# JasperSnoek/spearmint

Hardware: NVIDIA H100
Metric: EI candidates/sec (higher is better)
Workload: dtype f32

## Files before the change

### spearmint_b200/csrc/predict_tc.cu

```cuda
#include <cuda_fp16.h>
#include <cuda.h>

#include <algorithm>
#include <vector>
#include <cstdlib>
#include <cstring>

#include "common.cuh"
#include "tc_common.cuh"

namespace smk {

__global__ void __launch_bounds__(256, 2) trtri_finalize_kernel(int Npad, int ldx, int K, const float* __restrict__ winv,
                                                                 float* X) {
  using C = Cfg<float>;
  constexpr int NB = C::NB, TM = C::TM, TN = C::TN;
  extern __shared__ __align__(16) unsigned char smem_raw[];
  TileSmem<float>& sm = *reinterpret_cast<TileSmem<float>*>(smem_raw);
  float (*Ts)[NB + kPad] = reinterpret_cast<float (*)[NB + kPad]>(smem_raw + sizeof(TileSmem<float>));
  const int nblk = Npad / NB, J = blockIdx.x, s = blockIdx.y;
  const int tid = threadIdx.x, ty = tid >> 4, tx = tid & 15;
  const float* W = winv + ((long)s * nblk + K) * NB * NB;
  float* Xt = X + (long)s * ldx * ldx + (long)K * NB * ldx + (long)J * NB;
  float acc[TM][TN];
  if (J == K) {
#pragma unroll
    for (int r = 0; r < TM; ++r)
#pragma unroll
      for (int g = 0; g < TN / 4; ++g) {
        V4<float> v = ld4(W + (long)tile_row(ty, r) * NB + g * 64 + tx * 4);
#pragma unroll
        for (int e = 0; e < 4; ++e) acc[r][g * 4 + e] = v.v[e];
      }
  } else {
#pragma unroll
    for (int r = 0; r < TM; ++r)
#pragma unroll
      for (int g = 0; g < TN / 4; ++g) {
        V4<float> v = ld4(Xt + (long)tile_row(ty, r) * ldx + g * 64 + tx * 4);
        st4(&Ts[tile_row(ty, r)][g * 64 + tx * 4], v);
      }
#pragma unroll
    for (int r = 0; r < TM; ++r)
#pragma unroll
      for (int c = 0; c < TN; ++c) acc[r][c] = 0.f;
    TileGemm<float, Lay::KContig, Lay::MContig, false>::run_bsmem(acc, W, NB, &Ts[0][0], NB + kPad, NB, sm);
  }
#pragma unroll
  for (int r = 0; r < TM; ++r)
#pragma unroll
    for (int g = 0; g < TN / 4; ++g) {
      V4<float> v;
#pragma unroll
      for (int e = 0; e < 4; ++e) v.v[e] = acc[r][g * 4 + e];
      st4(Xt + (long)tile_row(ty, r) * ldx + g * 64 + tx * 4, v);
    }
}

__global__ void __launch_bounds__(256, 2) trtri_update_kernel(int Npad, int ldx, int K, const float* __restrict__ L,
                                                               float* X) {
  using C = Cfg<float>;
  constexpr int NB = C::NB, TM = C::TM, TN = C::TN;
  __shared__ TileSmem<float> sm;
  const int I = K + 1 + blockIdx.x, J = blockIdx.y, s = blockIdx.z;
  const int tid = threadIdx.x, ty = tid >> 4, tx = tid & 15;
  const float* Lik = L + (long)s * Npad * Npad + (long)I * NB * Npad + (long)K * NB;
  float* Xs = X + (long)s * ldx * ldx;
  float* Xij = Xs + (long)I * NB * ldx + (long)J * NB;
  const float* Xkj = Xs + (long)K * NB * ldx + (long)J * NB;
  float acc[TM][TN];
  if (K == J) {
#pragma unroll
    for (int r = 0; r < TM; ++r)
#pragma unroll
      for (int c = 0; c < TN; ++c) acc[r][c] = 0.f;
  } else {
#pragma unroll
    for (int r = 0; r < TM; ++r)
#pragma unroll
      for (int g = 0; g < TN / 4; ++g) {
        V4<float> v = ld4(Xij + (long)tile_row(ty, r) * ldx + g * 64 + tx * 4);
#pragma unroll
        for (int e = 0; e < 4; ++e) acc[r][g * 4 + e] = v.v[e];
      }
  }
  TileGemm<float, Lay::KContig, Lay::MContig, true>::run(acc, Lik, Npad, Xkj, ldx, NB, sm);
#pragma unroll
  for (int r = 0; r < TM; ++r)
#pragma unroll
    for (int g = 0; g < TN / 4; ++g) {
      V4<float> v;
#pragma unroll
      for (int e = 0; e < 4; ++e) v.v[e] = acc[r][g * 4 + e];
      st4(Xij + (long)tile_row(ty, r) * ldx + g * 64 + tx * 4, v);
    }
}

__device__ __forceinline__ float tf32_hi(float x) { return tf32_rn(x); }

__global__ void split_lower_kernel(int Npad, int ld, long total, const float* __restrict__ X, float* __restrict__ hi,
                                   float* __restrict__ lo) {
  long e = (long)blockIdx.x * blockDim.x + threadIdx.x;
  if (e >= total) return;
  long per = (long)ld * ld;
  int r = (int)((e % per) / ld), c = (int)(e % ld);
  float x = (c <= r && r < Npad) ? X[e] : 0.f;
  float h = tf32_hi(x);
  hi[e] = h;
  lo[e] = x - h;
}

__global__ void __launch_bounds__(256) linv_mv_kernel(int N, int Np, const float* __restrict__ hi,
                                                      const float* __restrict__ lo, const float* __restrict__ y,
                                                      const float* __restrict__ mean, float* __restrict__ t) {
  const int s = blockIdx.y, warp = threadIdx.x >> 5, lane = threadIdx.x & 31;
  const int row = blockIdx.x * 8 + warp;
  if (row >= Np) return;
  const long base = ((long)s * Np + row) * Np;
  const float mu = mean[s];
  float acc = 0.f;
  for (int k = lane; k <= row && k < N; k += 32) acc = fmaf(hi[base + k] + lo[base + k], y[k] - mu, acc);
#pragma unroll
  for (int o = 16; o > 0; o >>= 1) acc += __shfl_xor_sync(0xffffffffu, acc, o);
  if (lane == 0) t[(long)s * Np + row] = (row < N) ? acc : 0.f;
}
__global__ void __launch_bounds__(256) linv_mtv_kernel(int N, int Np, int ld_alpha, const float* __restrict__ hi,
                                                       const float* __restrict__ lo, const float* __restrict__ t,
                                                       float* __restrict__ alpha) {
  __shared__ float red[4][64];
  const int s = blockIdx.y, cl = threadIdx.x & 63, ph = threadIdx.x >> 6;
  const int c = blockIdx.x * 64 + cl;
  const float* th = t + (long)s * Np;
  const long base = (long)s * Np * Np + c;
  float acc = 0.f;
  if (c < N)
    for (int r = (c & ~3) + ph; r < N; r += 4)
      if (r >= c) acc = fmaf(hi[base + (long)r * Np] + lo[base + (long)r * Np], th[r], acc);
  red[ph][cl] = acc;
  __syncthreads();
  if (ph == 0 && c < ld_alpha) alpha[(long)s * ld_alpha + c] = (c < N) ? red[0][cl] + red[1][cl] + red[2][cl] + red[3][cl] : 0.f;
}

__global__ void __launch_bounds__(256) linv_absmax_kernel(long per4, const float4* __restrict__ hi,
                                                          const float4* __restrict__ lo, unsigned* __restrict__ maxbits) {
  const int s = blockIdx.y;
  const float4* h = hi + (long)s * per4;
  const float4* l = lo + (long)s * per4;
  float m = 0.f;
  for (long e = (long)blockIdx.x * blockDim.x + threadIdx.x; e < per4; e += (long)gridDim.x * blockDim.x) {
    float4 a = h[e], b = l[e];
    m = fmaxf(m, fmaxf(fmaxf(fabsf(a.x + b.x), fabsf(a.y + b.y)), fmaxf(fabsf(a.z + b.z), fabsf(a.w + b.w))));
  }
#pragma unroll
  for (int o = 16; o > 0; o >>= 1) m = fmaxf(m, __shfl_xor_sync(0xffffffffu, m, o));
  if ((threadIdx.x & 31) == 0) atomicMax(&maxbits[s], __float_as_uint(m));
}

__global__ void __launch_bounds__(256) linv_pack_f16_kernel(long per4, const float4* __restrict__ hi,
                                                            const float4* __restrict__ lo,
                                                            const unsigned* __restrict__ maxbits, uint2* __restrict__ oh,
                                                            uint2* __restrict__ ol, int* __restrict__ exps) {
  const int s = blockIdx.y;
  const int eb = scale_exp(__uint_as_float(maxbits[s]));
  const float sc = ldexpf(1.f, eb);
  if (blockIdx.x == 0 && threadIdx.x == 0) exps[s] = eb;
  const long base = (long)s * per4;
  for (long e = (long)blockIdx.x * blockDim.x + threadIdx.x; e < per4; e += (long)gridDim.x * blockDim.x) {
    float4 a = hi[base + e], b = lo[base + e];
    __half hh[4], ll[4];
    split16((a.x + b.x) * sc, hh[0], ll[0]);
    split16((a.y + b.y) * sc, hh[1], ll[1]);
    split16((a.z + b.z) * sc, hh[2], ll[2]);
    split16((a.w + b.w) * sc, hh[3], ll[3]);
    oh[base + e] = pack4(hh);
    ol[base + e] = pack4(ll);
  }
}

__global__ void __launch_bounds__(256) alpha_absmax_kernel(int N, int F, int Npad_alpha, const float* __restrict__ alpha,
                                                           int* __restrict__ fexp) {
  __shared__ float red[8];
  const int s = blockIdx.x;
  float m = 0.f;
  for (long e = threadIdx.x; e < (long)F * N; e += blockDim.x) {
    int f = (int)(e / N), n = (int)(e % N);
    m = fmaxf(m, fabsf(alpha[((long)s * F + f) * Npad_alpha + n]));
  }
#pragma unroll
  for (int o = 16; o > 0; o >>= 1) m = fmaxf(m, __shfl_xor_sync(0xffffffffu, m, o));
  if ((threadIdx.x & 31) == 0) red[threadIdx.x >> 5] = m;
  __syncthreads();
  if (threadIdx.x == 0) {
    for (int w = 1; w < 8; ++w) m = fmaxf(m, red[w]);
    fexp[s] = scale_exp(m);
  }
}
__global__ void alpha_pack_f16_kernel(int N, int Np, int F, int Fp, int Npad_alpha, long total,
                                      const float* __restrict__ alpha, const int* __restrict__ fexp,
                                      __half* __restrict__ hi, __half* __restrict__ lo) {
  long e = (long)blockIdx.x * blockDim.x + threadIdx.x;
  if (e >= total) return;
  int n = (int)(e % Np);
  long sf = e / Np;
  int f = (int)(sf % Fp), s = (int)(sf / Fp);
  float x = (f < F && n < N) ? alpha[((long)s * F + f) * Npad_alpha + n] * ldexpf(1.f, fexp[s]) : 0.f;
  split16(x, hi[e], lo[e]);
}

constexpr int kKD = 16;

__global__ void __launch_bounds__(256, 2) kxt_kernel(int kind, int N, int Np, int M, int c_begin, int Mc, int D,
                                                     const float* __restrict__ X, const float* __restrict__ Cc,
                                                     const float* __restrict__ inv_ls, const float* __restrict__ amp2,
                                                     const float* __restrict__ mean, const float* __restrict__ alpha,
                                                     int Npad_alpha, __half* __restrict__ khi,
                                                     __half* __restrict__ klo, float* __restrict__ mu, int ldm) {
  constexpr int T = 128, LDC = T + kPad, LDX = T + kPad;
  __shared__ __align__(16) float cs[kKD][LDC];
  __shared__ __align__(16) float xs[kKD][LDX];
  __shared__ __align__(16) float red[16][T];
  static_assert((LDC * sizeof(float)) % 16 == 0 && (LDX * sizeof(float)) % 16 == 0, "128-bit shared loads");
  const int s = blockIdx.y, c0 = blockIdx.x * T;
  const int tid = threadIdx.x, ty = tid >> 4, tx = tid & 15;
  const float* ils = inv_ls + (long)s * D;
  const float a2 = amp2[s];
  const float2 a2s = dup2(a2 * ldexpf(1.f, kx_exp(a2)));
  const float* al = alpha ? alpha + (long)s * Npad_alpha : nullptr;
  float2 mdot[8];
#pragma unroll
  for (int r = 0; r < 8; ++r) mdot[r] = make_float2(0.f, 0.f);

  for (int n0 = 0; n0 < Np; n0 += T) {
    float2 acc[8][4];
#pragma unroll
    for (int r = 0; r < 8; ++r)
#pragma unroll
      for (int c = 0; c < 4; ++c) acc[r][c] = make_float2(0.f, 0.f);
    for (int d0 = 0; d0 < D; d0 += kKD) {
      __syncthreads();
      for (int e = tid; e < T * kKD; e += 256) {
        int row = e / kKD, dd = e % kKD, d = d0 + dd;
        int gc = min(c_begin + c0 + row, M - 1), n = n0 + row;
        float sc = (d < D) ? ils[d] : 0.f;
        cs[dd][row] = (d < D) ? Cc[(long)gc * D + d] * sc : 0.f;
        xs[dd][row] = (d < D && n < N) ? -X[(long)n * D + d] * sc : 0.f;
      }
      __syncthreads();
      const int dmax = min(kKD, D - d0);
      for (int dd = 0; dd < dmax; ++dd) {
        float2 b[4];
#pragma unroll
        for (int g = 0; g < 2; ++g) {
          const V4<float> u = ld4(&xs[dd][g * 64 + tx * 4]);
          b[2 * g] = make_float2(u.v[0], u.v[1]);
          b[2 * g + 1] = make_float2(u.v[2], u.v[3]);
        }
#pragma unroll
        for (int g = 0; g < 2; ++g) {
          const float4 p0 = *reinterpret_cast<const float4*>(&cs[dd][g * 64 + ty * 4]);
          const float2 a[4] = {dup2(p0.x), dup2(p0.y), dup2(p0.z), dup2(p0.w)};
#pragma unroll
          for (int rr = 0; rr < 4; ++rr)
#pragma unroll
            for (int c = 0; c < 4; ++c) {
              const float2 df = fadd2(a[rr], b[c]);
              acc[g * 4 + rr][c] = ffma2(df, df, acc[g * 4 + rr][c]);
            }
        }
      }
    }
    const bool edge = (n0 + T > N);
    float2 av[4];
#pragma unroll
    for (int c = 0; c < 4; ++c) {
      const int n = n0 + (c >> 1) * 64 + tx * 4 + (c & 1) * 2;
      av[c] = al ? make_float2((n < N) ? al[n] : 0.f, (n + 1 < N) ? al[n + 1] : 0.f) : make_float2(0.f, 0.f);
    }
#pragma unroll
    for (int r = 0; r < 8; ++r) {
      const long ok = ((long)s * Mc + c0 + tile_row(ty, r)) * Np + n0;
#pragma unroll
      for (int g = 0; g < 2; ++g) {
        __half2 hh[2], ll[2];
#pragma unroll
        for (int q = 0; q < 2; ++q) {
          const int c = 2 * g + q;
          float2 kk = kernel_pair_fast(kind, acc[r][c]);
          if (edge) {
            const int n = n0 + g * 64 + tx * 4 + q * 2;
            if (n >= N) kk.x = 0.f;
            if (n + 1 >= N) kk.y = 0.f;
          }
          mdot[r] = ffma2(av[c], kk, mdot[r]);
          const float2 v = fmul2(kk, a2s);
          hh[q] = __floats2half2_rn(v.x, v.y);
          const float2 hf = __half22float2(hh[q]);
          ll[q] = __floats2half2_rn(v.x - hf.x, v.y - hf.y);
        }
        uint2 ph, pl;
        ph.x = *reinterpret_cast<unsigned*>(&hh[0]); ph.y = *reinterpret_cast<unsigned*>(&hh[1]);
        pl.x = *reinterpret_cast<unsigned*>(&ll[0]); pl.y = *reinterpret_cast<unsigned*>(&ll[1]);
        *reinterpret_cast<uint2*>(khi + ok + g * 64 + tx * 4) = ph;
        *reinterpret_cast<uint2*>(klo + ok + g * 64 + tx * 4) = pl;
      }
    }
  }
  if (!al) return;
  __syncthreads();
#pragma unroll
  for (int r = 0; r < 8; ++r) red[tx][tile_row(ty, r)] = mdot[r].x + mdot[r].y;
  __syncthreads();
  if (tid < T) {
    float v = 0.f;
    for (int q = 0; q < 16; ++q) v += red[q][tid];
    int gc = c_begin + c0 + tid;
    if (gc < M) mu[(long)s * ldm + gc] = fmaf(a2, v, mean[s]);
  }
}

namespace tc {
constexpr int BM = 128;
constexpr int BN = 256;
constexpr int BK = 16;
constexpr int BK16 = 32;
constexpr int STAGES = 4;
constexpr int ROW_BYTES = BK * 4;
static_assert(ROW_BYTES == 64 && BK16 * 2 == ROW_BYTES, "operand rows must be one 64B swizzle span in both element types");
constexpr int UK_BYTES = 32;
constexpr int A_BYTES = BM * ROW_BYTES;
constexpr int B_BYTES = BN * ROW_BYTES;
constexpr int STAGE_BYTES = 2 * A_BYTES + 2 * B_BYTES;
constexpr int CONSUMERS = 2;
constexpr int THREADS = (CONSUMERS + 1) * 128;
constexpr int PRODUCER_REGS = 40, CONSUMER_REGS = 232;
static_assert(128 * PRODUCER_REGS + CONSUMERS * 128 * CONSUMER_REGS <= 65536, "register file");
constexpr int SMEM_BYTES = STAGES * STAGE_BYTES + 1024  + 256 ;

struct Args {
  int S, Np, Mc, ntiles, npairs, ngroups, ldp;
  float* partial;
  const float* z;
  float* mpartial;
  float* dbg;
  int F, M, c_begin, ldm;
  const float* mean;
  float* mu_f;
  int f16;
  int a_evict_first;
  const float* amp2;
  const int* bexp;
  int mode;
  int Npad, jb, ncols;
  float* Cmat;
  int K;
  float *xhi, *xlo, *xthi, *xtlo;
};

struct Item { int valid, own, rowA, rowB, k0, nk, s, tile, g, pr; };

template <int CLUSTER>
__device__ __forceinline__ long num_items(const Args& p) {
  return p.mode <= 1 ? (long)p.S * ((p.ntiles + CLUSTER - 1) / CLUSTER) * p.npairs : (long)p.S * p.ntiles;
}
template <int CLUSTER>
__device__ __forceinline__ Item get_item(const Args& p, long w, int h, int rank) {
  Item it;
  it.valid = 0; it.own = 1; it.rowA = it.rowB = it.k0 = it.nk = it.s = it.tile = it.g = it.pr = 0;
  const int bk = p.f16 ? BK16 : BK;
  if (p.mode <= 1) {
    const int ntg = (p.ntiles + CLUSTER - 1) / CLUSTER;
    it.pr = (int)(w % p.npairs);
    const long st = w / p.npairs;
    it.tile = (int)(st % ntg) * CLUSTER + rank;
    it.s = (int)(st / ntg);
    if (it.tile >= p.ntiles) { it.tile = p.ntiles - 1; it.own = 0; }
    it.g = (h == 0) ? it.pr : p.ngroups - 1 - it.pr;
    if (h == 1 && (p.mode == 1 || it.g == it.pr)) return it;
    it.nk = (p.mode == 1) ? p.Np / bk : (it.g + 1) * (BN / bk);
    it.rowA = it.s * p.Mc + it.tile * BM;
    it.rowB = (it.s * p.ngroups + it.g) * BN;
    it.valid = 1;
  } else if (p.mode == 2) {
    if (h == 1) return it;
    it.tile = (int)(w % p.ntiles);
    it.s = (int)(w / p.ntiles);
    it.rowA = it.s * p.Npad + (p.jb + it.tile) * BM;
    it.rowB = it.s * p.Npad + p.jb * BM;
    it.nk = p.jb * BM / bk;
    it.valid = 1;
  } else {
    if (h == 1) return it;
    it.tile = (int)(w % p.ntiles);
    it.s = (int)(w / p.ntiles);
    it.rowA = it.s * BM;
    it.rowB = it.s * p.Np + it.tile * BN;
    it.k0 = it.tile * BN;
    it.nk = (p.K * BM - it.tile * BN) / bk;
    it.valid = 1;
  }
  return it;
}

template <int CLUSTER>
__global__ void __launch_bounds__(THREADS, 1)
predict_tc_kernel(const __grid_constant__ CUtensorMap mAhi, const __grid_constant__ CUtensorMap mAlo,
                  const __grid_constant__ CUtensorMap mBhi, const __grid_constant__ CUtensorMap mBlo, Args p) {
  static_assert(CLUSTER == 1 || CLUSTER == 2, "one CTA, or a pair sharing the B operand");
  extern __shared__ unsigned char smem_raw[];
  unsigned char* base = smem_raw + ((1024u - (smem_u32(smem_raw) & 1023u)) & 1023u);
  uint64_t* bars = reinterpret_cast<uint64_t*>(base + STAGES * STAGE_BYTES);
  uint64_t* full = bars;
  uint64_t* empty = bars + STAGES;

  const int warp = threadIdx.x >> 5, lane = threadIdx.x & 31;
  const int rank = CLUSTER > 1 ? (int)cluster_ctarank() : 0;
  if (threadIdx.x == 0) {
    for (int i = 0; i < STAGES; ++i) { mbar_init(&full[i], 1); mbar_init(&empty[i], CLUSTER * CONSUMERS * 4); }
    asm volatile("fence.mbarrier_init.release.cluster;" ::: "memory");
  }
  if (CLUSTER > 1) cluster_sync();
  else __syncthreads();

  const long nitems = num_items<CLUSTER>(p);
  const long w0 = blockIdx.x / CLUSTER, dw = gridDim.x / CLUSTER;
  const int bk = p.f16 ? BK16 : BK;
  if (warp < 4) {
    asm volatile("setmaxnreg.dec.sync.aligned.u32 %0;" ::"n"(PRODUCER_REGS));
    if (warp == 0 && lane == 0) {
      const uint64_t hintA = (p.mode == 0 && !p.a_evict_first) ? 0x1000000000000000ull : 0x12F0000000000000ull;
      const uint64_t hintB = 0x14F0000000000000ull;
      int stage = 0;
      uint32_t phase = 0;
      for (long w = w0; w < nitems; w += dw) {
        for (int h = 0; h < 2; ++h) {
          const Item it = get_item<CLUSTER>(p, w, h, rank);
          if (!it.valid) break;
          for (int kc = 0; kc < it.nk; ++kc) {
            mbar_wait_relaxed(&empty[stage], phase ^ 1, 64);
            unsigned char* sb = base + stage * STAGE_BYTES;
            const int kk = it.k0 + kc * bk;
            mbar_expect_tx(&full[stage], STAGE_BYTES);
            tma_load_2d(&mAhi, &full[stage], sb, kk, it.rowA, hintA);
            tma_load_2d(&mAlo, &full[stage], sb + A_BYTES, kk, it.rowA, hintA);
            if (CLUSTER == 1) {
              tma_load_2d(&mBhi, &full[stage], sb + 2 * A_BYTES, kk, it.rowB, hintB);
              tma_load_2d(&mBlo, &full[stage], sb + 2 * A_BYTES + B_BYTES, kk, it.rowB, hintB);
            } else {
              const int hb = rank * (BN / CLUSTER);
              const uint16_t all = (1u << CLUSTER) - 1;
              tma_load_2d_multicast(&mBhi, &full[stage], sb + 2 * A_BYTES + hb * ROW_BYTES, kk, it.rowB + hb, all, hintB);
              tma_load_2d_multicast(&mBlo, &full[stage], sb + 2 * A_BYTES + B_BYTES + hb * ROW_BYTES, kk, it.rowB + hb,
                                    all, hintB);
            }
            if (++stage == STAGES) { stage = 0; phase ^= 1; }
          }
        }
      }
    }
    if (CLUSTER > 1) cluster_sync();
    return;
  }

  asm volatile("setmaxnreg.inc.sync.aligned.u32 %0;" ::"n"(CONSUMER_REGS));
  const int wg = (warp >> 2) - 1;
  const int r0 = wg * 64 + (warp & 3) * 16 + (lane >> 2);
  const int cq = 2 * (lane & 3);
  const uint32_t a_off = (uint32_t)wg * 64 * ROW_BYTES;
  auto release = [&](int st) {
    if (CLUSTER == 1) mbar_arrive(&empty[st]);
    else
#pragma unroll
      for (int r = 0; r < CLUSTER; ++r) mbar_arrive_cluster(&empty[st], r);
  };
  float d[BN / 2];
  int stage = 0;
  uint32_t phase = 0;
  for (long w = w0; w < nitems; w += dw) {
    float acc[2] = {0.f, 0.f}, accm[2] = {0.f, 0.f};
    const Item it0 = get_item<CLUSTER>(p, w, 0, rank);
    for (int h = 0; h < 2; ++h) {
      const Item it = get_item<CLUSTER>(p, w, h, rank);
      if (!it.valid) break;
      int prev = -1;
      for (int kc = 0; kc < it.nk; ++kc) {
        mbar_wait(&full[stage], phase);
        const uint32_t sa = smem_u32(base + stage * STAGE_BYTES);
        const uint64_t ahi = wgmma_desc_sw64(sa + a_off), alo = wgmma_desc_sw64(sa + A_BYTES + a_off);
        const uint64_t bhi = wgmma_desc_sw64(sa + 2 * A_BYTES), blo = wgmma_desc_sw64(sa + 2 * A_BYTES + B_BYTES);
        wgmma_fence();
        if (p.f16) {
#pragma unroll
          for (int k = 0; k < ROW_BYTES / UK_BYTES; ++k) {
            const uint64_t ko = (uint64_t)((k * UK_BYTES) >> 4);
            wgmma_f16_n256(d, alo + ko, bhi + ko, (kc | k) ? 1u : 0u);
            wgmma_f16_n256(d, ahi + ko, blo + ko, 1u);
            wgmma_f16_n256(d, ahi + ko, bhi + ko, 1u);
          }
        } else {
#pragma unroll
          for (int k = 0; k < ROW_BYTES / UK_BYTES; ++k) {
            const uint64_t ko = (uint64_t)((k * UK_BYTES) >> 4);
            wgmma_tf32_n256(d, alo + ko, bhi + ko, (kc | k) ? 1u : 0u);
            wgmma_tf32_n256(d, ahi + ko, blo + ko, 1u);
            wgmma_tf32_n256(d, ahi + ko, bhi + ko, 1u);
          }
        }
        wgmma_commit();
        wgmma_wait<1>();
        if (prev >= 0 && lane == 0) release(prev);
        prev = stage;
        if (++stage == STAGES) { stage = 0; phase ^= 1; }
      }
      wgmma_wait<0>();
      wgmma_hold(d);
      if (prev >= 0 && lane == 0) release(prev);
      if (!it.own) continue;
      const float scl = p.f16 ? ldexpf(1.f, -(kx_exp(p.amp2[it.s]) + p.bexp[it.s])) : 1.f;
      if (p.mode == 0) {
        const float* zrow = p.z ? p.z + (long)it.s * p.Np + it.g * BN : nullptr;
#pragma unroll
        for (int nb = 0; nb < BN / 8; ++nb) {
          const int c = nb * 8 + cq;
          const float2 z2 = zrow ? __ldg(reinterpret_cast<const float2*>(zrow + c)) : make_float2(0.f, 0.f);
#pragma unroll
          for (int rh = 0; rh < 2; ++rh) {
            const float v0 = d[nb * 4 + rh * 2] * scl, v1 = d[nb * 4 + rh * 2 + 1] * scl;
            acc[rh] = fmaf(v0, v0, acc[rh]);
            acc[rh] = fmaf(v1, v1, acc[rh]);
            accm[rh] = fmaf(v0, z2.x, accm[rh]);
            accm[rh] = fmaf(v1, z2.y, accm[rh]);
            if (p.dbg) {
              float* o = p.dbg + ((long)it.s * p.Mc + it.tile * BM + r0 + 8 * rh) * p.Np + it.g * BN + c;
              o[0] = v0;
              o[1] = v1;
            }
          }
        }
      } else if (p.mode == 1) {
        const float mu0 = p.mean[it.s];
#pragma unroll
        for (int rh = 0; rh < 2; ++rh) {
          const int gc = p.c_begin + it.tile * BM + r0 + 8 * rh;
          if (gc >= p.M) continue;
#pragma unroll
          for (int nb = 0; nb < BN / 8; ++nb)
#pragma unroll
// ... 77 lines not shown
    return;
  }
  if (nmp > 0) {
    float m = 0.f;
    for (int j = 0; j < nmp; ++j) m += mu_partial[((long)j * S + s) * ldp + c];
    mu[(long)s * ldm + c_begin + c] = fmaf(amp2[s], m, mean[s]);
  }
}

}
__global__ void kxt_mu_finish_kernel(int M, int Mc, int S, int nmp, const float* __restrict__ mu_partial,
                                     const float* __restrict__ amp2, const float* __restrict__ mean,
                                     float* __restrict__ mu, int ldm) {
  int c = blockIdx.x * blockDim.x + threadIdx.x, s = blockIdx.y;
  if (c >= M) return;
  float m = 0.f;
  for (int j = 0; j < nmp; ++j) m += mu_partial[((long)j * S + s) * Mc + c];
  mu[(long)s * ldm + c] = fmaf(amp2[s], m, mean[s]);
}
int num_sms();
namespace tc {

typedef CUresult (*EncodeTiledFn)(CUtensorMap*, CUtensorMapDataType, cuuint32_t, void*, const cuuint64_t*,
                                  const cuuint64_t*, const cuuint32_t*, const cuuint32_t*, CUtensorMapInterleave,
                                  CUtensorMapSwizzle, CUtensorMapL2promotion, CUtensorMapFloatOOBfill);

static EncodeTiledFn encode_fn() {
  static EncodeTiledFn fn = nullptr;
  if (!fn) {
    void* p = nullptr;
    cudaDriverEntryPointQueryResult q;
    if (cudaGetDriverEntryPoint("cuTensorMapEncodeTiled", &p, cudaEnableDefault, &q) == cudaSuccess) fn = (EncodeTiledFn)p;
  }
  return fn;
}

static int make_map(CUtensorMap* m, const float* ptr, uint64_t rows, uint64_t cols, uint32_t box_rows) {
  EncodeTiledFn f = encode_fn();
  if (!f) return 1;
  cuuint64_t dims[2] = {cols, rows};
  cuuint64_t strides[1] = {cols * sizeof(float)};
  cuuint32_t box[2] = {(cuuint32_t)BK, box_rows};
  cuuint32_t estr[2] = {1, 1};
  CUresult r = f(m, CU_TENSOR_MAP_DATA_TYPE_FLOAT32, 2, const_cast<float*>(ptr), dims, strides, box, estr,
                 CU_TENSOR_MAP_INTERLEAVE_NONE, CU_TENSOR_MAP_SWIZZLE_64B, CU_TENSOR_MAP_L2_PROMOTION_L2_256B,
                 CU_TENSOR_MAP_FLOAT_OOB_FILL_NONE);
  return r == CUDA_SUCCESS ? 0 : 2;
}
static int make_map_h(CUtensorMap* m, const __half* ptr, uint64_t rows, uint64_t cols, uint32_t box_rows) {
  EncodeTiledFn f = encode_fn();
  if (!f) return 1;
  cuuint64_t dims[2] = {cols, rows};
  cuuint64_t strides[1] = {cols * sizeof(__half)};
  cuuint32_t box[2] = {(cuuint32_t)BK16, box_rows};
  cuuint32_t estr[2] = {1, 1};
  CUresult r = f(m, CU_TENSOR_MAP_DATA_TYPE_FLOAT16, 2, const_cast<__half*>(ptr), dims, strides, box, estr,
                 CU_TENSOR_MAP_INTERLEAVE_NONE, CU_TENSOR_MAP_SWIZZLE_64B, CU_TENSOR_MAP_L2_PROMOTION_L2_256B,
                 CU_TENSOR_MAP_FLOAT_OOB_FILL_NONE);
  return r == CUDA_SUCCESS ? 0 : 2;
}

constexpr int kPredictCluster = 2;
static int launch_predict(const CUtensorMap& mAhi, const CUtensorMap& mAlo, const CUtensorMap& mBhi,
                          const CUtensorMap& mBlo, const Args& a, cudaStream_t st) {
  constexpr int C = kPredictCluster;
  auto kern = predict_tc_kernel<C>;
  static int max_clusters = 0;
  cudaLaunchConfig_t cfg = {};
  cudaLaunchAttribute attr[1];
  attr[0].id = cudaLaunchAttributeClusterDimension;
  attr[0].val.clusterDim.x = C;
  attr[0].val.clusterDim.y = 1;
  attr[0].val.clusterDim.z = 1;
  cfg.blockDim = dim3(THREADS);
  cfg.dynamicSmemBytes = SMEM_BYTES;
  cfg.stream = st;
  cfg.attrs = attr;
  cfg.numAttrs = 1;
  if (!max_clusters) {
    cudaError_t e = cudaFuncSetAttribute(kern, cudaFuncAttributeMaxDynamicSharedMemorySize, SMEM_BYTES);
    cfg.gridDim = dim3(C * num_sms());
    if (e == cudaSuccess) e = cudaOccupancyMaxActiveClusters(&max_clusters, kern, &cfg);
    if (e != cudaSuccess || max_clusters <= 0) {
      max_clusters = 0;
      return check_launch("predict_tc cluster occupancy");
    }
  }
  const long nitems = (long)a.S * ((a.ntiles + C - 1) / C) * a.npairs;
  cfg.gridDim = dim3((unsigned)(std::min<long>(nitems, max_clusters) * C));
  cudaLaunchKernelEx(&cfg, kern, mAhi, mAlo, mBhi, mBlo, a);
  return check_launch("predict_tc_kernel");
}
}
bool kxt_tc_supported(int D, int S);
bool kxt_tc_preferred(int D, int S);
int kxt_tc_ngroups(int Np);
size_t kxt_tc_workspace_bytes(int Np, int Mc, int S, int M, int D);
int kxt_tc_prepare(void* ws, int N, int Np, int M, int Mc, int D, int S, const float* X, const float* Cc, cudaStream_t st);
int kxt_tc(void* ws, int kind, int N, int Np, int M, int c_begin, int Mc, int mc_used, int D, int S, const float* inv_ls,
           const float* amp2, const float* alpha, int Npad_alpha, __half* khi, __half* klo, cudaStream_t st);
float* kxt_tc_mu_partial(void* ws, int Np, int Mc, int S, int M, int D);
static const int kKxtWsD = 32;

int tc_np(int N) { return ((N + tc::BN - 1) / tc::BN) * tc::BN; }

size_t trtri_workspace_bytes(int Np, int S) { return (size_t)S * Np * Np * sizeof(float); }

int trtri_split(int Npad, int Np, int S, const float* L, const float* winv, float* linv_hi, float* linv_lo,
                void* workspace, size_t workspace_bytes, cudaStream_t st) {
  if (Npad <= 0 || Npad % kNpadMult) return -1;
  if (Np < Npad || Np % tc::BN) return -2;
  if (S <= 0) return -3;
  if (!L || !winv || !linv_hi || !linv_lo) return -4;
  if (!workspace || workspace_bytes < trtri_workspace_bytes(Np, S)) return -8;
  float* X = reinterpret_cast<float*>(workspace);
  const size_t dsm = sizeof(TileSmem<float>) + sizeof(float) * 128 * (128 + kPad);
  static bool attr = false;
  if (!attr) {
    cudaFuncSetAttribute(trtri_finalize_kernel, cudaFuncAttributeMaxDynamicSharedMemorySize, (int)dsm);
    attr = true;
  }
  const int nblk = Npad / 128;
  timing_begin("trtri_kernel", st);
  for (int K = 0; K < nblk; ++K) {
    trtri_finalize_kernel<<<dim3(K + 1, S), 256, dsm, st>>>(Npad, Np, K, winv, X);
    if (K + 1 < nblk) trtri_update_kernel<<<dim3(nblk - K - 1, K + 1, S), 256, 0, st>>>(Npad, Np, K, L, X);
  }
  timing_end(st);
  count_launch(2 * nblk - 1);
  const long total = (long)S * Np * Np;
  split_lower_kernel<<<(unsigned)((total + 255) / 256), 256, 0, st>>>(Npad, Np, total, X, linv_hi, linv_lo);
  count_launch(1);
  return check_launch("trtri_split");
}

static void tc_args_init(tc::Args& a) {
  memset(&a, 0, sizeof(a));
}

int tc_chol_update(int Npad, int S, int jb, int ncols, float* A, const float* lhi, const float* llo, cudaStream_t st) {
  CUtensorMap mAhi, mAlo, mBhi, mBlo;
  if (tc::make_map(&mAhi, lhi, (uint64_t)S * Npad, Npad, tc::BM) || tc::make_map(&mAlo, llo, (uint64_t)S * Npad, Npad, tc::BM) ||
      tc::make_map(&mBhi, lhi, (uint64_t)S * Npad, Npad, tc::BN) || tc::make_map(&mBlo, llo, (uint64_t)S * Npad, Npad, tc::BN))
    return 1999;
  static bool attr = false;
  if (!attr) {
    cudaFuncSetAttribute(tc::predict_tc_kernel<1>, cudaFuncAttributeMaxDynamicSharedMemorySize, tc::SMEM_BYTES);
    attr = true;
  }
  tc::Args a;
  tc_args_init(a);
  a.mode = 2; a.S = S; a.Npad = Npad; a.jb = jb; a.ncols = ncols; a.Cmat = A;
  a.ntiles = Npad / tc::BM - jb; a.npairs = 1; a.ngroups = 1;
  long nitems = (long)S * a.ntiles;
  int grid = (int)std::min<long>(nitems, num_sms());
  timing_begin("tc_chol_update", st);
  tc::predict_tc_kernel<1><<<grid, tc::THREADS, tc::SMEM_BYTES, st>>>(mAhi, mAlo, mBhi, mBlo, a);
  timing_end(st);
  count_launch();
  return check_launch("tc_chol_update");
}

__global__ void __launch_bounds__(256, 2) trtri_lt_kernel(int Npad, int K, const float* __restrict__ L,
                                                           const float* __restrict__ winv, float* __restrict__ lthi,
                                                           float* __restrict__ ltlo) {
  using C = Cfg<float>;
  constexpr int NB = C::NB, TM = C::TM, TN = C::TN;
  __shared__ TileSmem<float> sm;
  const int nblk = Npad / NB, J = blockIdx.x, s = blockIdx.y;
  const int tid = threadIdx.x, ty = tid >> 4, tx = tid & 15;
  const float* W = winv + ((long)s * nblk + K) * NB * NB;
  const float* Lk = L + (long)s * Npad * Npad + (long)K * NB * Npad + (long)J * NB;
  float acc[TM][TN];
#pragma unroll
  for (int r = 0; r < TM; ++r)
#pragma unroll
    for (int c = 0; c < TN; ++c) acc[r][c] = 0.f;
  TileGemm<float, Lay::KContig, Lay::MContig, false>::run(acc, W, NB, Lk, Npad, NB, sm);
  const long off = (long)s * NB * Npad + (long)J * NB;
#pragma unroll
  for (int r = 0; r < TM; ++r)
#pragma unroll
    for (int g = 0; g < TN / 4; ++g) {
      V4<float> h, l;
#pragma unroll
      for (int e = 0; e < 4; ++e) {
        float x = acc[r][g * 4 + e];
        h.v[e] = tf32_hi(x);
        l.v[e] = tf32_lo(x, h.v[e]);
      }
      const long o = off + (long)tile_row(ty, r) * Npad + g * 64 + tx * 4;
      st4(lthi + o, h);
      st4(ltlo + o, l);
    }
}

__global__ void trtri_diag_store_kernel(int Npad, int Np, int K, const float* __restrict__ winv, float* __restrict__ xhi,
                                        float* __restrict__ xlo, float* __restrict__ xthi, float* __restrict__ xtlo) {
  constexpr int NB = 128;
  const int s = blockIdx.y, nblk = Npad / NB;
  const float* W = winv + ((long)s * nblk + K) * NB * NB;
  for (int e = blockIdx.x * blockDim.x + threadIdx.x; e < NB * NB; e += gridDim.x * blockDim.x) {
    int i = e / NB, k = e % NB;
    float x = W[e], h = tf32_hi(x), l = x - h;
    long o = ((long)s * Np + (long)K * NB + i) * Np + (long)K * NB + k;
    long ot = ((long)s * Np + (long)K * NB + k) * Np + (long)K * NB + i;
    xhi[o] = h; xlo[o] = l; xthi[ot] = h; xtlo[ot] = tf32_lo(x, h);
  }
}

size_t trtri_tc_workspace_bytes(int Npad, int Np, int S) {
  return (2 * (size_t)S * Np * Np + 2 * (size_t)S * 128 * Npad) * sizeof(float);
}

int potrf_lower_batched_tc(int, int, float*, float*, int*, float*, float*, cudaStream_t, cudaEvent_t*);
void potrf_winv_block(int, int, int, const float*, float*, cudaStream_t);

static int trtri_tc_run(int Npad, int Np, int S, const float* L, float* winv, float* linv_hi, float* linv_lo,
                        void* workspace, size_t workspace_bytes, cudaStream_t st, cudaEvent_t* blk_done) {
  if (Npad <= 0 || Npad % kNpadMult) return -1;
  if (Np < Npad || Np % tc::BN) return -2;
  if (S <= 0) return -3;
  if (!L || !winv || !linv_hi || !linv_lo) return -4;
  if (!workspace || workspace_bytes < trtri_tc_workspace_bytes(Npad, Np, S)) return -8;
  float* xthi = reinterpret_cast<float*>(workspace);
  float* xtlo = xthi + (size_t)S * Np * Np;
  float* lthi = xtlo + (size_t)S * Np * Np;
  float* ltlo = lthi + (size_t)S * 128 * Npad;
  const size_t xb = (size_t)S * Np * Np * sizeof(float);
  cudaMemsetAsync(linv_hi, 0, xb, st);
  cudaMemsetAsync(linv_lo, 0, xb, st);
  cudaMemsetAsync(xthi, 0, 2 * xb, st);
  CUtensorMap mAhi, mAlo, mBhi, mBlo;
  if (tc::make_map(&mAhi, lthi, (uint64_t)S * 128, Npad, tc::BM) || tc::make_map(&mAlo, ltlo, (uint64_t)S * 128, Npad, tc::BM) ||
      tc::make_map(&mBhi, xthi, (uint64_t)S * Np, Np, tc::BN) || tc::make_map(&mBlo, xtlo, (uint64_t)S * Np, Np, tc::BN))
    return 1999;
  static bool attr = false;
  if (!attr) {
    cudaFuncSetAttribute(tc::predict_tc_kernel<1>, cudaFuncAttributeMaxDynamicSharedMemorySize, tc::SMEM_BYTES);
    attr = true;
  }
  const int nblk = Npad / 128;
  timing_begin("trtri_kernel", st);
  for (int K = 0; K < nblk; ++K) {
    if (blk_done) {
      cudaStreamWaitEvent(st, blk_done[K], 0);
      potrf_winv_block(Npad, S, K, L, winv, st);
    }
    trtri_diag_store_kernel<<<dim3(8, S), 256, 0, st>>>(Npad, Np, K, winv, linv_hi, linv_lo, xthi, xtlo);
    count_launch();
    if (K == 0) continue;
    trtri_lt_kernel<<<dim3(K, S), 256, 0, st>>>(Npad, K, L, winv, lthi, ltlo);
    tc::Args a;
    tc_args_init(a);
    a.mode = 3; a.S = S; a.Np = Np; a.Npad = Npad; a.K = K;
    a.ntiles = (K * 128 + tc::BN - 1) / tc::BN; a.npairs = 1; a.ngroups = 1;
    a.xhi = linv_hi; a.xlo = linv_lo; a.xthi = xthi; a.xtlo = xtlo;
    long nitems = (long)S * a.ntiles;
    int grid = (int)std::min<long>(nitems, num_sms());
    tc::predict_tc_kernel<1><<<grid, tc::THREADS, tc::SMEM_BYTES, st>>>(mAhi, mAlo, mBhi, mBlo, a);
    count_launch(2);
  }
  timing_end(st);
  return check_launch("trtri_split_tc");
}

int trtri_split_tc(int Npad, int Np, int S, const float* L, const float* winv, float* linv_hi, float* linv_lo,
                   void* workspace, size_t workspace_bytes, cudaStream_t st) {
  return trtri_tc_run(Npad, Np, S, L, const_cast<float*>(winv), linv_hi, linv_lo, workspace, workspace_bytes, st, nullptr);
}

int potrf_trtri_tc(int Npad, int Np, int S, float* A, float* winv, int* info, float* lhi, float* llo, float* linv_hi,
                   float* linv_lo, void* tws, size_t tws_bytes, cudaStream_t st) {
  if (Npad <= 0 || Npad % kNpadMult) return -1;
  static cudaStream_t aux = nullptr;
  static cudaEvent_t ev_in = nullptr, ev_out = nullptr;
  static std::vector<cudaEvent_t> blk;
  if (!aux) {
    cudaStreamCreateWithFlags(&aux, cudaStreamNonBlocking);
    cudaEventCreateWithFlags(&ev_in, cudaEventDisableTiming);
    cudaEventCreateWithFlags(&ev_out, cudaEventDisableTiming);
  }
  const int nblk = Npad / 128;
  while ((int)blk.size() < nblk) {
    cudaEvent_t e;
    cudaEventCreateWithFlags(&e, cudaEventDisableTiming);
    blk.push_back(e);
  }
  cudaEventRecord(ev_in, st);
  cudaStreamWaitEvent(aux, ev_in, 0);
  int rc = potrf_lower_batched_tc(Npad, S, A, winv, info, lhi, llo, st, blk.data());
  if (rc) return rc;
  rc = trtri_tc_run(Npad, Np, S, A, winv, linv_hi, linv_lo, tws, tws_bytes, aux, blk.data());
  cudaEventRecord(ev_out, aux);
  cudaStreamWaitEvent(st, ev_out, 0);
  return rc;
}

int linv_pack_f16(int Np, int S, const float* linv_hi, const float* linv_lo, __half* out_hi, __half* out_lo, int* exps,
                  cudaStream_t st) {
  if (Np <= 0 || Np % tc::BN) return -1;
  if (S <= 0) return -2;
  if (!linv_hi || !linv_lo || !out_hi || !out_lo || !exps) return -3;
  unsigned* maxbits = reinterpret_cast<unsigned*>(exps + S);
  cudaMemsetAsync(maxbits, 0, sizeof(unsigned) * S, st);
  const long per4 = (long)Np * Np / 4;
  const int gx = (int)std::min<long>((per4 + 255) / 256, 4L * num_sms());
  timing_begin("linv_pack_f16", st);
  linv_absmax_kernel<<<dim3(gx, S), 256, 0, st>>>(per4, reinterpret_cast<const float4*>(linv_hi),
                                                  reinterpret_cast<const float4*>(linv_lo), maxbits);
  linv_pack_f16_kernel<<<dim3(gx, S), 256, 0, st>>>(per4, reinterpret_cast<const float4*>(linv_hi),
                                                    reinterpret_cast<const float4*>(linv_lo), maxbits,
                                                    reinterpret_cast<uint2*>(out_hi), reinterpret_cast<uint2*>(out_lo), exps);
  timing_end(st);
  count_launch(2);
  return check_launch("linv_pack_f16");
}

int linv_alpha(int N, int Np, int S, const float* linv_hi, const float* linv_lo, const float* y, const float* mean,
               float* alpha, int ld_alpha, float* tmp, cudaStream_t st) {
  if (N <= 0 || Np < N) return -1;
  if (S <= 0) return -3;
  if (!linv_hi || !linv_lo || !y || !mean || !alpha || !tmp) return -4;
  if (ld_alpha < N) return -9;
  linv_mv_kernel<<<dim3((Np + 7) / 8, S), 256, 0, st>>>(N, Np, linv_hi, linv_lo, y, mean, tmp);
  linv_mtv_kernel<<<dim3((ld_alpha + 63) / 64, S), 256, 0, st>>>(N, Np, ld_alpha, linv_hi, linv_lo, tmp, alpha);
  count_launch(2);
  return check_launch("linv_alpha");
}

static bool tc_overlap_enabled() {
  static int v = -1;
  if (v < 0) { const char* e = getenv("SMK_TC_OVERLAP"); v = (e && e[0] == '1') ? 1 : 0; }
  return v == 1;
}
static size_t tc_chunk_cands(int Np, int M, int S, size_t budget) {
  size_t per_cand = (size_t)S * Np * 2 * sizeof(__half);
  size_t mpad = ((size_t)M + 127) / 128 * 128;
  size_t mc = budget / per_cand;
  if (mc >= mpad) return mpad;
  if (tc_overlap_enabled()) mc = (budget / 2) / per_cand;
  mc = mc / 128 * 128;
  if (mc < 128) mc = 128;
  return mc;
}
static int tc_nbuf(int Np, int M, int S, size_t budget) {
  size_t mpad = ((size_t)M + 127) / 128 * 128;
  if (!tc_overlap_enabled()) return 1;
  return tc_chunk_cands(Np, M, S, budget) >= mpad ? 1 : 2;
}
static size_t tc_budget() {
  const char* e = getenv("SMK_TC_BUDGET_MB");
  if (e && e[0]) { long mb = atol(e); if (mb > 0) return (size_t)mb << 20; }
  return (size_t)20 << 30;
}
#define kTcBudget (tc_budget())

static int fant_rows(int F) { return F > 1 ? ((F + tc::BN - 1) / tc::BN) * tc::BN : 0; }

size_t predict_tc_workspace_bytes(int Np, int M, int S, int F) {
  size_t mc = tc_chunk_cands(Np, M, S, kTcBudget);
  int ngroups = Np / tc::BN, npairs = (ngroups + 1) / 2, nbuf = tc_nbuf(Np, M, S, kTcBudget);
  return (size_t)nbuf * S * mc * Np * 2 * sizeof(__half) + 2 * (size_t)npairs * S * mc * sizeof(float) +
         2 * (size_t)S * fant_rows(F) * Np * sizeof(__half) + (size_t)S * sizeof(int) + 1024 +
         kxt_tc_workspace_bytes(Np, (int)mc, S, M, kKxtWsD);
}

size_t kxt_pack_workspace_bytes(int Np, int M, int S) {
  return kxt_tc_workspace_bytes(Np, ((M + 127) / 128) * 128, S, M, kKxtWsD) + 256;
}
int kxt_pack(int impl, int kind, int N, int Np, int M, int D, int S, const float* X, const float* Cc, const float* inv_ls,
             const float* amp2, const float* mean, const float* alpha, int Npad_alpha, __half* khi, __half* klo,
             float* mu, int ldm, void* workspace, size_t workspace_bytes, cudaStream_t st) {
  if (kind < 0 || kind > 3) return -2;
  if (N <= 0 || Np < N || Np % tc::BN) return -4;
  if (M <= 0 || D <= 0 || S <= 0) return -5;
  if (!X || !Cc || !inv_ls || !amp2 || !mean || !alpha || !khi || !klo || !mu) return -8;
  if (ldm < M) return -18;
  const int Mc = ((M + 127) / 128) * 128;
  if (impl == 0) {
    kxt_kernel<<<dim3(Mc / 128, S), 256, 0, st>>>(kind, N, Np, M, 0, Mc, D, X, Cc, inv_ls, amp2, mean, alpha, Npad_alpha,
                                                  khi, klo, mu, ldm);
    count_launch();
    return check_launch("kxt_pack");
  }
  if (!kxt_tc_supported(D, S)) return -1;
  if (!workspace || workspace_bytes < kxt_pack_workspace_bytes(Np, M, S)) return -20;
  const int nmp = kxt_tc_ngroups(Np);
  int rc = kxt_tc_prepare(workspace, N, Np, M, Mc, D, S, X, Cc, st);
  if (rc) return rc;
  rc = kxt_tc(workspace, kind, N, Np, M, 0, Mc, Mc, D, S, inv_ls, amp2, alpha, Npad_alpha, khi, klo, st);
  if (rc) return rc;
  float* mu_partial = kxt_tc_mu_partial(workspace, Np, Mc, S, M, D);
  kxt_mu_finish_kernel<<<dim3((Mc + 255) / 256, S), 256, 0, st>>>(M, Mc, S, nmp, mu_partial, amp2, mean, mu, ldm);
  count_launch();
  return check_launch("kxt_pack");
}

struct PregenState {
  bool valid = false;
  void* ws = nullptr;
  int M = 0, S = 0, Np = 0, N = 0;
  cudaEvent_t done = nullptr, fork = nullptr;
  cudaStream_t stream = nullptr;
};
static PregenState g_pregen;

int predict_tc_pregen(int kind, int N, int Np, int M, int D, int S, const float* X, const float* Cc, const float* inv_ls,
                      const float* amp2, void* workspace, size_t workspace_bytes, int F, cudaStream_t st) {
  if (kind < 0 || kind > 3) return -1;
  if (N <= 0 || Np < N || Np % tc::BN) return -3;
  if (M <= 0 || D <= 0 || S <= 0) return -4;
  if (!X || !Cc || !inv_ls || !amp2) return -7;
  const bool fant = F > 1;
  if (!workspace || workspace_bytes < predict_tc_workspace_bytes(Np, M, S, fant ? F : 1)) return -20;
  if (tc_nbuf(Np, M, S, kTcBudget) != 1) return -22;
  const int Mc = (int)tc_chunk_cands(Np, M, S, kTcBudget);
  const int ngroups = Np / tc::BN, npairs = (ngroups + 1) / 2;
  const size_t kelems = (size_t)S * Mc * Np;
  __half* kbase = reinterpret_cast<__half*>(workspace);
  float* partial = reinterpret_cast<float*>(kbase + 2 * kelems);
  const int Fp = fant ? fant_rows(F) : 0;
  __half* ahi = reinterpret_cast<__half*>(partial + 2 * (size_t)npairs * S * Mc);
  int* fexp = reinterpret_cast<int*>(ahi + 2 * (size_t)S * Fp * Np);
  void* kws = reinterpret_cast<void*>(fexp + S);
  static int gen_env = -1;
  if (gen_env < 0) { const char* e = getenv("SMK_KXT_IMPL"); gen_env = (e && !strcmp(e, "tc")) ? 1 : 0; }
  const bool gen_tc = gen_env == 1 && kxt_tc_preferred(D, S);
  PregenState& g = g_pregen;
  if (!g.stream) {
    cudaStreamCreateWithFlags(&g.stream, cudaStreamNonBlocking);
    cudaEventCreateWithFlags(&g.done, cudaEventDisableTiming);
    cudaEventCreateWithFlags(&g.fork, cudaEventDisableTiming);
  }
  cudaEventRecord(g.fork, st);
  cudaStreamWaitEvent(g.stream, g.fork, 0);
  const int mc_used = min(Mc, (M + 127) / 128 * 128);
  timing_begin("kxt_kernel", g.stream);
  if (gen_tc) {
    int rc = kxt_tc_prepare(kws, N, Np, M, Mc, D, S, X, Cc, g.stream);
    if (rc) return rc;
    rc = kxt_tc(kws, kind, N, Np, M, 0, Mc, mc_used, D, S, inv_ls, amp2, nullptr, 0, kbase, kbase + kelems, g.stream);
    if (rc) return rc;
  } else {
    kxt_kernel<<<dim3(mc_used / 128, S), 256, 0, g.stream>>>(kind, N, Np, M, 0, Mc, D, X, Cc, inv_ls, amp2, nullptr, nullptr, 0,
                                                             kbase, kbase + kelems, nullptr, 0);
    count_launch();
  }
  timing_end(g.stream);
  cudaEventRecord(g.done, g.stream);
  g.valid = true; g.ws = workspace; g.M = M; g.S = S; g.Np = Np; g.N = N;
  return check_launch("predict_tc_pregen");
}

int predict_tc(int kind, int N, int Np, int M, int D, int S, const float* X, const float* Cc, const float* inv_ls,
               const float* amp2, const float* mean, const __half* linv_hi, const __half* linv_lo, const int* linv_exp,
               const float* alpha, int Npad_alpha, float* mu, float* var, int ldm, void* workspace,
               size_t workspace_bytes, float* dbg, int F, const float* alpha_f, float* mu_f, const float* z,
               int pregenerated, cudaStream_t st) {
  if (kind < 0 || kind > 3) return -1;
  if (N <= 0) return -2;
  if (Np < N || Np % tc::BN) return -3;
  if (M <= 0) return -4;
  if (D <= 0) return -5;
// ... 124 lines not shown
```

Baseline: 216,800.

## Pipeline trtri across priority streams and skip zero triangles in linv packing

The trtri spine (diag store and lt kernels) moves to a high-priority stream, and a double-buffered lt workspace lets block K+1's lt overlap the mode-3 GEMM of block K. Factorization gets its own high-priority stream. Full memsets are replaced by a kernel that zeroes only the region above the diagonal blocks. The linv absmax and pack kernels walk rows and read only the lower-triangular prefix, writing zeros elsewhere. TC grids now launch one CTA per work item with a tile-major order instead of capping at the SM count. These changes target serialization, redundant memory traffic and launch underuse, in exchange for more streams, events and workspace.

```diff
diff --git a/spearmint_b200/csrc/predict_tc.cu b/spearmint_b200/csrc/predict_tc.cu
--- a/spearmint_b200/csrc/predict_tc.cu
+++ b/spearmint_b200/csrc/predict_tc.cu
@@ -141,39 +141,51 @@
   if (ph == 0 && c < ld_alpha) alpha[(long)s * ld_alpha + c] = (c < N) ? red[0][cl] + red[1][cl] + red[2][cl] + red[3][cl] : 0.f;
 }
 
-__global__ void __launch_bounds__(256) linv_absmax_kernel(long per4, const float4* __restrict__ hi,
+__device__ __forceinline__ int linv_prefix4(int r) { return ((r >> 8) + 1) * 64; }
+
+__global__ void __launch_bounds__(256) linv_absmax_kernel(int Np, const float4* __restrict__ hi,
                                                           const float4* __restrict__ lo, unsigned* __restrict__ maxbits) {
-  const int s = blockIdx.y;
-  const float4* h = hi + (long)s * per4;
-  const float4* l = lo + (long)s * per4;
+  const int s = blockIdx.y, np4 = Np / 4;
   float m = 0.f;
-  for (long e = (long)blockIdx.x * blockDim.x + threadIdx.x; e < per4; e += (long)gridDim.x * blockDim.x) {
-    float4 a = h[e], b = l[e];
-    m = fmaxf(m, fmaxf(fmaxf(fabsf(a.x + b.x), fabsf(a.y + b.y)), fmaxf(fabsf(a.z + b.z), fabsf(a.w + b.w))));
+  for (int r = blockIdx.x; r < Np; r += gridDim.x) {
+    const long row = ((long)s * Np + r) * np4;
+    const int n4 = linv_prefix4(r);
+    for (int e = threadIdx.x; e < n4; e += blockDim.x) {
+      float4 a = hi[row + e], b = lo[row + e];
+      m = fmaxf(m, fmaxf(fmaxf(fabsf(a.x + b.x), fabsf(a.y + b.y)), fmaxf(fabsf(a.z + b.z), fabsf(a.w + b.w))));
+    }
   }
 #pragma unroll
   for (int o = 16; o > 0; o >>= 1) m = fmaxf(m, __shfl_xor_sync(0xffffffffu, m, o));
   if ((threadIdx.x & 31) == 0) atomicMax(&maxbits[s], __float_as_uint(m));
 }
 
-__global__ void __launch_bounds__(256) linv_pack_f16_kernel(long per4, const float4* __restrict__ hi,
+__global__ void __launch_bounds__(256) linv_pack_f16_kernel(int Np, const float4* __restrict__ hi,
                                                             const float4* __restrict__ lo,
                                                             const unsigned* __restrict__ maxbits, uint2* __restrict__ oh,
                                                             uint2* __restrict__ ol, int* __restrict__ exps) {
-  const int s = blockIdx.y;
+  const int s = blockIdx.y, np4 = Np / 4;
   const int eb = scale_exp(__uint_as_float(maxbits[s]));
   const float sc = ldexpf(1.f, eb);
   if (blockIdx.x == 0 && threadIdx.x == 0) exps[s] = eb;
-  const long base = (long)s * per4;
-  for (long e = (long)blockIdx.x * blockDim.x + threadIdx.x; e < per4; e += (long)gridDim.x * blockDim.x) {
-    float4 a = hi[base + e], b = lo[base + e];
-    __half hh[4], ll[4];
-    split16((a.x + b.x) * sc, hh[0], ll[0]);
-    split16((a.y + b.y) * sc, hh[1], ll[1]);
-    split16((a.z + b.z) * sc, hh[2], ll[2]);
-    split16((a.w + b.w) * sc, hh[3], ll[3]);
-    oh[base + e] = pack4(hh);
-    ol[base + e] = pack4(ll);
+  for (int r = blockIdx.x; r < Np; r += gridDim.x) {
+    const long row = ((long)s * Np + r) * np4;
+    const int n4 = linv_prefix4(r);
+    for (int e = threadIdx.x; e < np4; e += blockDim.x) {
+      if (e >= n4) {
+        oh[row + e] = make_uint2(0u, 0u);
+        ol[row + e] = make_uint2(0u, 0u);
+        continue;
+      }
+      float4 a = hi[row + e], b = lo[row + e];
+      __half hh[4], ll[4];
+      split16((a.x + b.x) * sc, hh[0], ll[0]);
+      split16((a.y + b.y) * sc, hh[1], ll[1]);
+      split16((a.z + b.z) * sc, hh[2], ll[2]);
+      split16((a.w + b.w) * sc, hh[3], ll[3]);
+      oh[row + e] = pack4(hh);
+      ol[row + e] = pack4(ll);
+    }
   }
 }
 
@@ -390,8 +402,8 @@
     it.valid = 1;
   } else {
     if (h == 1) return it;
-    it.tile = (int)(w % p.ntiles);
-    it.s = (int)(w / p.ntiles);
+    it.tile = (int)(w / p.S);
+    it.s = (int)(w % p.S);
     it.rowA = it.s * BM;
     it.rowB = it.s * p.Np + it.tile * BN;
     it.k0 = it.tile * BN;
@@ -775,10 +787,8 @@
   tc_args_init(a);
   a.mode = 2; a.S = S; a.Npad = Npad; a.jb = jb; a.ncols = ncols; a.Cmat = A;
   a.ntiles = Npad / tc::BM - jb; a.npairs = 1; a.ngroups = 1;
-  long nitems = (long)S * a.ntiles;
-  int grid = (int)std::min<long>(nitems, num_sms());
   timing_begin("tc_chol_update", st);
-  tc::predict_tc_kernel<1><<<grid, tc::THREADS, tc::SMEM_BYTES, st>>>(mAhi, mAlo, mBhi, mBlo, a);
+  tc::predict_tc_kernel<1><<<S * a.ntiles, tc::THREADS, tc::SMEM_BYTES, st>>>(mAhi, mAlo, mBhi, mBlo, a);
   timing_end(st);
   count_launch();
   return check_launch("tc_chol_update");
@@ -832,8 +842,24 @@
   }
 }
 
+__global__ void __launch_bounds__(256) trtri_zero_kernel(int Npad, int Np, float* __restrict__ xhi, float* __restrict__ xlo,
+                                                         float* __restrict__ xthi, float* __restrict__ xtlo) {
+  const int r = blockIdx.x, s = blockIdx.y;
+  const long row = ((long)s * Np + r) * Np;
+  const float4 z = make_float4(0.f, 0.f, 0.f, 0.f);
+  for (int c = (r < Npad ? (r / 128 + 1) * 128 : 0) + 4 * threadIdx.x; c < Np; c += 4 * blockDim.x) {
+    *reinterpret_cast<float4*>(xhi + row + c) = z;
+    *reinterpret_cast<float4*>(xlo + row + c) = z;
+  }
+  if ((r & 255) >= 128 && threadIdx.x < 32) {
+    const long o = row + (r & ~255) + 4 * threadIdx.x;
+    *reinterpret_cast<float4*>(xthi + o) = z;
+    *reinterpret_cast<float4*>(xtlo + o) = z;
+  }
+}
+
 size_t trtri_tc_workspace_bytes(int Npad, int Np, int S) {
-  return (2 * (size_t)S * Np * Np + 2 * (size_t)S * 128 * Npad) * sizeof(float);
+  return (2 * (size_t)S * Np * Np + 4 * (size_t)S * 128 * Npad) * sizeof(float);
 }
 
 int potrf_lower_batched_tc(int, int, float*, float*, int*, float*, float*, cudaStream_t, cudaEvent_t*);
@@ -846,44 +872,70 @@
   if (S <= 0) return -3;
   if (!L || !winv || !linv_hi || !linv_lo) return -4;
   if (!workspace || workspace_bytes < trtri_tc_workspace_bytes(Npad, Np, S)) return -8;
+  const int nblk = Npad / 128;
+  static cudaStream_t spine = nullptr;
+  static cudaEvent_t ev_in = nullptr, ev_spine = nullptr;
+  static std::vector<cudaEvent_t> ev_lt, ev_m3;
+  if (!spine) {
+    int lo = 0, hi = 0;
+    cudaDeviceGetStreamPriorityRange(&lo, &hi);
+    cudaStreamCreateWithPriority(&spine, cudaStreamNonBlocking, hi);
+    cudaEventCreateWithFlags(&ev_in, cudaEventDisableTiming);
+    cudaEventCreateWithFlags(&ev_spine, cudaEventDisableTiming);
+  }
+  while ((int)ev_lt.size() < nblk) {
+    cudaEvent_t e, f;
+    cudaEventCreateWithFlags(&e, cudaEventDisableTiming);
+    cudaEventCreateWithFlags(&f, cudaEventDisableTiming);
+    ev_lt.push_back(e);
+    ev_m3.push_back(f);
+  }
   float* xthi = reinterpret_cast<float*>(workspace);
   float* xtlo = xthi + (size_t)S * Np * Np;
-  float* lthi = xtlo + (size_t)S * Np * Np;
-  float* ltlo = lthi + (size_t)S * 128 * Npad;
-  const size_t xb = (size_t)S * Np * Np * sizeof(float);
-  cudaMemsetAsync(linv_hi, 0, xb, st);
-  cudaMemsetAsync(linv_lo, 0, xb, st);
-  cudaMemsetAsync(xthi, 0, 2 * xb, st);
-  CUtensorMap mAhi, mAlo, mBhi, mBlo;
-  if (tc::make_map(&mAhi, lthi, (uint64_t)S * 128, Npad, tc::BM) || tc::make_map(&mAlo, ltlo, (uint64_t)S * 128, Npad, tc::BM) ||
-      tc::make_map(&mBhi, xthi, (uint64_t)S * Np, Np, tc::BN) || tc::make_map(&mBlo, xtlo, (uint64_t)S * Np, Np, tc::BN))
+  float* lt[2][2];
+  for (int b = 0; b < 2; ++b)
+    for (int h = 0; h < 2; ++h) lt[b][h] = xtlo + (size_t)S * Np * Np + (size_t)(2 * b + h) * S * 128 * Npad;
+  CUtensorMap mAhi[2], mAlo[2], mBhi, mBlo;
+  for (int b = 0; b < 2; ++b)
+    if (tc::make_map(&mAhi[b], lt[b][0], (uint64_t)S * 128, Npad, tc::BM) ||
+        tc::make_map(&mAlo[b], lt[b][1], (uint64_t)S * 128, Npad, tc::BM))
+      return 1999;
+  if (tc::make_map(&mBhi, xthi, (uint64_t)S * Np, Np, tc::BN) || tc::make_map(&mBlo, xtlo, (uint64_t)S * Np, Np, tc::BN))
     return 1999;
   static bool attr = false;
   if (!attr) {
     cudaFuncSetAttribute(tc::predict_tc_kernel<1>, cudaFuncAttributeMaxDynamicSharedMemorySize, tc::SMEM_BYTES);
     attr = true;
   }
-  const int nblk = Npad / 128;
+  cudaEventRecord(ev_in, st);
+  cudaStreamWaitEvent(spine, ev_in, 0);
+  trtri_zero_kernel<<<dim3(Np, S), 256, 0, st>>>(Npad, Np, linv_hi, linv_lo, xthi, xtlo);
+  count_launch();
   timing_begin("trtri_kernel", st);
   for (int K = 0; K < nblk; ++K) {
     if (blk_done) {
-      cudaStreamWaitEvent(st, blk_done[K], 0);
-      potrf_winv_block(Npad, S, K, L, winv, st);
-    }
-    trtri_diag_store_kernel<<<dim3(8, S), 256, 0, st>>>(Npad, Np, K, winv, linv_hi, linv_lo, xthi, xtlo);
+      cudaStreamWaitEvent(spine, blk_done[K], 0);
+      potrf_winv_block(Npad, S, K, L, winv, spine);
+    }
+    trtri_diag_store_kernel<<<dim3(8, S), 256, 0, spine>>>(Npad, Np, K, winv, linv_hi, linv_lo, xthi, xtlo);
     count_launch();
     if (K == 0) continue;
-    trtri_lt_kernel<<<dim3(K, S), 256, 0, st>>>(Npad, K, L, winv, lthi, ltlo);
+    const int b = K & 1;
+    if (K >= 3) cudaStreamWaitEvent(spine, ev_m3[K - 2], 0);
+    trtri_lt_kernel<<<dim3(K, S), 256, 0, spine>>>(Npad, K, L, winv, lt[b][0], lt[b][1]);
+    cudaEventRecord(ev_lt[K], spine);
+    cudaStreamWaitEvent(st, ev_lt[K], 0);
     tc::Args a;
     tc_args_init(a);
     a.mode = 3; a.S = S; a.Np = Np; a.Npad = Npad; a.K = K;
     a.ntiles = (K * 128 + tc::BN - 1) / tc::BN; a.npairs = 1; a.ngroups = 1;
     a.xhi = linv_hi; a.xlo = linv_lo; a.xthi = xthi; a.xtlo = xtlo;
-    long nitems = (long)S * a.ntiles;
-    int grid = (int)std::min<long>(nitems, num_sms());
-    tc::predict_tc_kernel<1><<<grid, tc::THREADS, tc::SMEM_BYTES, st>>>(mAhi, mAlo, mBhi, mBlo, a);
+    tc::predict_tc_kernel<1><<<S * a.ntiles, tc::THREADS, tc::SMEM_BYTES, st>>>(mAhi[b], mAlo[b], mBhi, mBlo, a);
+    cudaEventRecord(ev_m3[K], st);
     count_launch(2);
   }
+  cudaEventRecord(ev_spine, spine);
+  cudaStreamWaitEvent(st, ev_spine, 0);
   timing_end(st);
   return check_launch("trtri_split_tc");
 }
@@ -896,12 +948,16 @@
 int potrf_trtri_tc(int Npad, int Np, int S, float* A, float* winv, int* info, float* lhi, float* llo, float* linv_hi,
                    float* linv_lo, void* tws, size_t tws_bytes, cudaStream_t st) {
   if (Npad <= 0 || Npad % kNpadMult) return -1;
-  static cudaStream_t aux = nullptr;
-  static cudaEvent_t ev_in = nullptr, ev_out = nullptr;
+  static cudaStream_t fac = nullptr, aux = nullptr;
+  static cudaEvent_t ev_in = nullptr, ev_fac = nullptr, ev_out = nullptr;
   static std::vector<cudaEvent_t> blk;
   if (!aux) {
-    cudaStreamCreateWithFlags(&aux, cudaStreamNonBlocking);
+    int lo = 0, hi = 0;
+    cudaDeviceGetStreamPriorityRange(&lo, &hi);
+    cudaStreamCreateWithPriority(&fac, cudaStreamNonBlocking, hi);
+    cudaStreamCreateWithPriority(&aux, cudaStreamNonBlocking, lo);
     cudaEventCreateWithFlags(&ev_in, cudaEventDisableTiming);
+    cudaEventCreateWithFlags(&ev_fac, cudaEventDisableTiming);
     cudaEventCreateWithFlags(&ev_out, cudaEventDisableTiming);
   }
   const int nblk = Npad / 128;
@@ -911,11 +967,14 @@
     blk.push_back(e);
   }
   cudaEventRecord(ev_in, st);
+  cudaStreamWaitEvent(fac, ev_in, 0);
   cudaStreamWaitEvent(aux, ev_in, 0);
-  int rc = potrf_lower_batched_tc(Npad, S, A, winv, info, lhi, llo, st, blk.data());
+  int rc = potrf_lower_batched_tc(Npad, S, A, winv, info, lhi, llo, fac, blk.data());
   if (rc) return rc;
   rc = trtri_tc_run(Npad, Np, S, A, winv, linv_hi, linv_lo, tws, tws_bytes, aux, blk.data());
+  cudaEventRecord(ev_fac, fac);
   cudaEventRecord(ev_out, aux);
+  cudaStreamWaitEvent(st, ev_fac, 0);
   cudaStreamWaitEvent(st, ev_out, 0);
   return rc;
 }
@@ -927,12 +986,11 @@
   if (!linv_hi || !linv_lo || !out_hi || !out_lo || !exps) return -3;
   unsigned* maxbits = reinterpret_cast<unsigned*>(exps + S);
   cudaMemsetAsync(maxbits, 0, sizeof(unsigned) * S, st);
-  const long per4 = (long)Np * Np / 4;
-  const int gx = (int)std::min<long>((per4 + 255) / 256, 4L * num_sms());
+  const int gx = std::min(Np, std::max(1, 8 * num_sms() / S));
   timing_begin("linv_pack_f16", st);
-  linv_absmax_kernel<<<dim3(gx, S), 256, 0, st>>>(per4, reinterpret_cast<const float4*>(linv_hi),
+  linv_absmax_kernel<<<dim3(gx, S), 256, 0, st>>>(Np, reinterpret_cast<const float4*>(linv_hi),
                                                   reinterpret_cast<const float4*>(linv_lo), maxbits);
-  linv_pack_f16_kernel<<<dim3(gx, S), 256, 0, st>>>(per4, reinterpret_cast<const float4*>(linv_hi),
+  linv_pack_f16_kernel<<<dim3(gx, S), 256, 0, st>>>(Np, reinterpret_cast<const float4*>(linv_hi),
                                                     reinterpret_cast<const float4*>(linv_lo), maxbits,
                                                     reinterpret_cast<uint2*>(out_hi), reinterpret_cast<uint2*>(out_lo), exps);
   timing_end(st);
```

New measurement: 221,400 (median of 6 runs). +2.1%, better.
